# smallflyingpig/speech-to-image-translation-without-text

Measured on AMD Instinct MI355X. Metric: StackGAN-v2 3-stage G+D train-step images/sec at 256px, higher is better.
Workload: dtype f32

## Files before the change

include/s2i_hip.h:

```cpp
#ifndef S2I_HIP_H
#define S2I_HIP_H

#include <stddef.h>
#include <stdint.h>

#ifdef __cplusplus
extern "C" {
#endif

#define S2I_ABI_VERSION 4

#define S2I_CONV_K1      0
#define S2I_CONV_K3S1    1
#define S2I_CONV_K4S2    2
#define S2I_TCONV_K4S2   3

#define S2I_CONV_1D      4

#define S2I_ACT_NONE     0
#define S2I_ACT_GLU      1
#define S2I_ACT_LRELU    2
#define S2I_ACT_TANH     3
#define S2I_ACT_RELU     4

// ... 145 lines not shown
                    long long* num_batches_tracked , float momentum,
                    float eps, float* out4, void* stream);
int s2i_bn_eval_coeffs(int C, const float* gamma, const float* beta, const float* running_mean,
                       const float* running_var, float eps, float* out4, void* stream);
int s2i_bn_act_forward(const float* y, long long M, int groups, int C, const float* coef4, int act,
                       const float* residual, float* out, void* stream);
int s2i_colstats(const float* y, long long M, int C, int ldy, float* part, int nparts,
                 void* stream);
int s2i_bn_act_bwd_reduce(const float* y, const float* dout, int lddout, long long M, int groups, int C,
                          const float* coef4, int act, float* part, int nparts, void* stream);
int s2i_bn_bwd_finalize(const float* part, int nparts, int groups, int C, long long count, float* dgamma,
                        float* dbeta, int accumulate, float* red2, void* stream);
int s2i_bn_act_bwd_apply(const float* y, const float* dout, int lddout, long long M, int groups, int C,
                         const float* coef4, const float* red2, int act, float* dy, void* stream);

int s2i_act_backward(const float* out, const float* dout, int lddout, long long M, int C, int act,
                     float* dy, void* stream);
int s2i_glu_forward(const float* x, long long M, int C, float* out, void* stream);
int s2i_glu_backward(const float* x, const float* dout, long long M, int C, float* dx,
                     void* stream);

int s2i_nchw_to_nhwc(const float* src, float* dst, int B, int C, int H, int W, int Cp,
                     void* stream);
int s2i_nhwc_to_nchw(const float* src, int lds, float* dst, int B, int C, int H, int W,
                     void* stream);
int s2i_image_to_u8(const float* src, int lds, unsigned char* dst, long long npix, void* stream);
int s2i_u8_to_image(const unsigned char* src, float* dst, int B, int H, int W, void* stream);
int s2i_image_batch(const unsigned char* pool, long long pool_bytes, const long long* offsets, const int* sizes,
                    int npool, const int* plan, int n, int S, int L, const int* tab1, const int* tab2, float* out0,
                    float* out1, float* out2, void* stream);
// ... 112 lines not shown
```

speech_to_image_translation_without_text_amd/_lib.py:

```python
import ctypes
import os

import torch

_HERE = os.path.dirname(os.path.abspath(__file__))
LIB_PATH = os.path.join(_HERE, "libs2i_hip.so")

CONV_K1, CONV_K3S1, CONV_K4S2, TCONV_K4S2, CONV_1D = 0, 1, 2, 3, 4
ACT_NONE, ACT_GLU, ACT_LRELU, ACT_TANH, ACT_RELU = 0, 1, 2, 3, 4
PACK_PLAIN, PACK_UPFOLD = 0, 1
DT_F32, DT_BF16 = 0, 1
POOL_MAX3S2, POOL_AVG3S1, POOL_GLOBAL = 0, 1, 2
POOL_THEN_LRN, LRN_THEN_POOL = 0, 1
LOGMEL_BFT, LOGMEL_NHWC = 0, 1
LOGMEL_TILE_FRAMES = 64
ABI_VERSION = 4

c_int, c_float, c_void_p, c_size_t, c_ll = (ctypes.c_int, ctypes.c_float, ctypes.c_void_p,
                                            ctypes.c_size_t, ctypes.c_longlong)


class ConvDesc(ctypes.Structure):
    _fields_ = [(n, c_int) for n in ("kind", "B", "H", "W", "Cx", "Cc", "N", "wmode", "flip", "wR",
                                     "ldw", "act", "stats", "ldy", "groups", "nosplit", "kw", "stride", "pad",
# ... 63 lines not shown
    "s2i_cvec_bias_table": (c_int, [P, P, c_int, c_int, c_int, c_int, c_int, P, P, c_size_t, P]),
    "s2i_border_sums_workspace_bytes": (c_size_t, [c_int, c_int, c_int, c_int]),
    "s2i_tap_sums": (c_int, [P, c_int, c_int, c_int, c_int, P, P, c_size_t, P]),
    "s2i_cvec_grads": (c_int, [P, P, P, c_int, c_int, c_int, c_int, c_int, c_int, c_int, P, P, c_int, P]),
    "s2i_wgrad_workspace_bytes": (c_size_t, [ctypes.POINTER(WgradDesc)]),
    "s2i_conv_wgrad": (c_int, [ctypes.POINTER(WgradDesc), P, P, P, P, P, c_size_t, P]),
    "s2i_pack_conv_weight": (c_int, [P, P, c_int, c_int, c_int, c_int, c_int, c_int, P]),
    "s2i_pack_conv_weights_batched": (c_int, [P, c_int, c_int, c_int, P]),
    "s2i_bn_finalize": (c_int, [P, c_int, c_int, c_int, c_ll, P, P, P, P, P, c_float, c_float, P, P]),
    "s2i_bn_eval_coeffs": (c_int, [c_int, P, P, P, P, c_float, P, P]),
    "s2i_bn_act_forward": (c_int, [P, c_ll, c_int, c_int, P, c_int, P, P, P]),
    "s2i_colstats": (c_int, [P, c_ll, c_int, c_int, P, c_int, P]),
    "s2i_bn_act_bwd_reduce": (c_int, [P, P, c_int, c_ll, c_int, c_int, P, c_int, P, c_int, P]),
    "s2i_bn_bwd_finalize": (c_int, [P, c_int, c_int, c_int, c_ll, P, P, c_int, P, P]),
    "s2i_bn_act_bwd_apply": (c_int, [P, P, c_int, c_ll, c_int, c_int, P, P, c_int, P, P]),
    "s2i_act_backward": (c_int, [P, P, c_int, c_ll, c_int, c_int, P, P]),
    "s2i_glu_forward": (c_int, [P, c_ll, c_int, P, P]),
    "s2i_glu_backward": (c_int, [P, P, c_ll, c_int, P, P]),
    "s2i_nchw_to_nhwc": (c_int, [P, P, c_int, c_int, c_int, c_int, c_int, P]),
    "s2i_nhwc_to_nchw": (c_int, [P, c_int, P, c_int, c_int, c_int, c_int, P]),
    "s2i_image_to_u8": (c_int, [P, c_int, P, c_ll, P]),
    "s2i_u8_to_image": (c_int, [P, P, c_int, c_int, c_int, P]),
    "s2i_image_batch": (c_int, [P, c_ll, P, P, c_int, P, c_int, c_int, c_int, P, P, P, P, P, P]),
    "s2i_spatial_sum": (c_int, [P, c_int, c_int, c_int, c_int, P, P, c_size_t, P]),
    "s2i_spatial_sum_workspace_bytes": (c_size_t, [c_int, c_int, c_int]),
    "s2i_reparam_forward": (c_int, [P, P, c_int, c_int, P, P]),
    "s2i_reparam_backward": (c_int, [P, P, P, P, P, c_int, c_int, P, P]),
    "s2i_kl_forward": (c_int, [P, c_int, P, c_int, c_int, c_int, P, P]),
    "s2i_kl_backward": (c_int, [P, c_int, P, c_int, c_int, c_int, P, P, P, P]),
    "s2i_logit_forward": (c_int, [P, P, P, c_int, c_int, P, P]),
# ... 56 lines not shown
        fn = getattr(lib, name)
        fn.restype = res
        fn.argtypes = args
    if lib.s2i_version() != ABI_VERSION:
        raise S2IError("libs2i_hip.so ABI version %d, expected %d: rebuild it (make -C csrc)" % (lib.s2i_version(), ABI_VERSION))
    _lib = lib
    return lib


def check(rc, what):
    if rc != 0:
        msg = load().s2i_last_error()
        raise S2IError("%s failed: %s" % (what, msg.decode() if msg else "unknown error"))


class tuning:

    def __init__(self, **knobs):
        self.knobs = knobs

    def __enter__(self):
        lib = load()
        self.old = {}
        for k, v in self.knobs.items():
            cur = c_int(0)
            check(lib.s2i_get_tuning(k.encode(), ctypes.byref(cur)), "s2i_get_tuning")
            self.old[k] = cur.value
            check(lib.s2i_set_tuning(k.encode(), int(v)), "s2i_set_tuning")
        return self

    def __exit__(self, *exc):
        lib = load()
        for k, v in self.old.items():
            check(lib.s2i_set_tuning(k.encode(), v), "s2i_set_tuning")
        return False


def require_device():
    global _device_checked
    if _device_checked:
        return
    if not torch.cuda.is_available():
        raise S2IError("no HIP device visible: the MI355X kernels have no CPU fallback")
    check(load().s2i_check_device(), "s2i_check_device")
    _device_checked = True


def ptr(t):
    if t is None:
# ... 15 lines not shown
```

speech_to_image_translation_without_text_amd/csrc/s2i_bn.hip:

```cpp
#include "s2i_elementwise.h"

namespace {
template <typename T>
__device__ __forceinline__ f32x4 act_dz(const T* __restrict__ y, const T* __restrict__ dout, int lddout,
                                        long long row, int C, int quad, const float* __restrict__ coef,
                                        int act, f32x4 yv) {
  const float* scale = coef + 2 * C;
  const float* shift = coef + 3 * C;
  f32x4 dz;
  if (act == S2I_ACT_GLU) {
    const int hq = C / 8;
    const bool first = quad < hq;
    const int pq = first ? quad + hq : quad - hq;
    const f32x4 yp = ld4(y + row * C + pq * 4);
    const f32x4 d = ld4(dout + row * lddout + (first ? quad : pq) * 4);
    const f32x4 sa = ld4(scale + (first ? quad : pq) * 4), ta = ld4(shift + (first ? quad : pq) * 4);
    const f32x4 sg = ld4(scale + (first ? pq : quad) * 4), tg = ld4(shift + (first ? pq : quad) * 4);
    const f32x4 ya = first ? yv : yp, yg = first ? yp : yv;
#pragma unroll
    for (int j = 0; j < 4; ++j) {
      const float za = sa[j] * ya[j] + ta[j];
      const float sgm = sigmoid_gate_<T>(sg[j] * yg[j] + tg[j]);
      dz[j] = first ? d[j] * sgm : d[j] * za * sgm * (1.f - sgm);
    }
// ... 752 lines not shown
  }
}
}
extern "C" int s2i_glu_forward(const float* x, long long M, int C, float* out, void* stream) {
  S2I_REQUIRE(x && out && M > 0 && C > 0 && C % 2 == 0, "glu_forward: bad args");
  hipLaunchKernelGGL(glu_fwd_kernel, dim3(grid_for(M * (C / 2))), dim3(256), 0, ST, x, M, C, out);
  S2I_LAUNCH_CHECK("glu_forward");
  return 0;
}
extern "C" int s2i_glu_backward(const float* x, const float* dout, long long M, int C, float* dx, void* stream) {
  S2I_REQUIRE(x && dout && dx && M > 0 && C > 0 && C % 2 == 0, "glu_backward: bad args");
  hipLaunchKernelGGL(glu_bwd_kernel, dim3(grid_for(M * (C / 2))), dim3(256), 0, ST, x, dout, M, C, dx);
  S2I_LAUNCH_CHECK("glu_backward");
  return 0;
}
```

speech_to_image_translation_without_text_amd/csrc/s2i_common.h:

```cpp
#pragma once
#include <hip/hip_runtime.h>
#include <stdio.h>
#include <stdarg.h>
#include "../../include/s2i_hip.h"

typedef float f32x16 __attribute__((ext_vector_type(16)));
typedef float f32x4 __attribute__((ext_vector_type(4)));

void s2i_set_error(const char* fmt, ...);

#define S2I_FAIL(...)            \
  do {                           \
    s2i_set_error(__VA_ARGS__);  \
    return 1;                    \
  } while (0)

#define S2I_REQUIRE(cond, ...)   \
  do {                           \
    if (!(cond)) S2I_FAIL(__VA_ARGS__); \
  } while (0)

#define S2I_LAUNCH_CHECK(name)                                          \
  do {                                                                  \
    hipError_t e__ = hipGetLastError();                                 \
// ... 5 lines not shown
  while ((1 << l) < v) ++l;
  return l;
}
static inline bool s2i_is_pow2(int v) { return v > 0 && (v & (v - 1)) == 0; }
static inline int s2i_cdiv(long long a, long long b) { return (int)((a + b - 1) / b); }

enum {
  S2I_TUNE_FWD_BM = 0,
  S2I_TUNE_FWD_MIN_CPS,
  S2I_TUNE_B16_V2,
  S2I_TUNE_B16_PERSIST,
  S2I_TUNE_FINALIZE_THREADS,
  S2I_TUNE_B16_DBG,
  S2I_TUNE_WGRAD16_BM,
  S2I_TUNE_WGRAD_BM,
  S2I_TUNE_COUNT
};
int s2i_tune(int key, int def);
```

speech_to_image_translation_without_text_amd/csrc/s2i_conv.hip:

```cpp
#include "s2i_igemm.h"

namespace {

static int fwd_splitk(long long blocks, int nchunks, int nosplit, int min_cps) {
  int splitk = 1;
  if (blocks < 512 && nchunks >= 16 && !nosplit) {
    splitk = (int)(768 / blocks);
    if (splitk > nchunks / min_cps) splitk = nchunks / min_cps;
    if (splitk > 64) splitk = 64;
    if (splitk < 1) splitk = 1;
  }
  return splitk;
}

int plan_fwd(const s2i_conv_desc* d, FwdPlan* pl) {
  S2I_REQUIRE(d->B > 0 && d->H > 0 && d->W > 0 && d->N > 0, "conv: non-positive extent");
  S2I_REQUIRE(d->Cx >= 0 && d->Cc >= 0 && (d->Cx % 4) == 0 && (d->Cc % 4) == 0 && d->Cx + d->Cc > 0,
              "conv: channel counts must be multiples of 4 (Cx=%d Cc=%d)", d->Cx, d->Cc);
  S2I_REQUIRE(s2i_is_pow2(d->H) && s2i_is_pow2(d->W), "conv: spatial extents must be powers of two");
  pl->Ca = d->Cx + d->Cc;
  pl->nphases = 1;
  switch (d->kind) {
    case S2I_CONV_K1: pl->T = 1; pl->Ho = d->H; pl->Wo = d->W; break;
    case S2I_CONV_K3S1: pl->T = 9; pl->Ho = d->H; pl->Wo = d->W; break;
// ... 83 lines not shown
    if (ppg < 1) ppg = 1;
    return ppg * groups;
  }
  return pl.gridM * pl.nphases;
}

extern "C" int s2i_conv_stat_parts(const s2i_conv_desc* d) {
  FwdPlan pl;
  if (plan_fwd(d, &pl)) return -1;
  return stat_parts_for(pl, d->groups);
}

static int conv_forward_impl(const s2i_conv_desc* d, const float* x, const float* cvec, const float* w,
                             const unsigned short* wsp, int planes, int np, int kp, const float* bias,
                             const float* cls_bias, float* y, float* part, void* ws, size_t ws_bytes, void* stream,
                             int x16 = 0, int y16 = 0, const float* in_coef = nullptr) {
  FwdPlan pl;
  if (plan_fwd(d, &pl)) return 1;
  S2I_REQUIRE(!cls_bias || (d->kind == S2I_CONV_K3S1 && pl.splitk == 1), "conv: class bias needs an unsplit 3x3 conv");
  S2I_REQUIRE(x != nullptr || d->Cx == 0, "conv: x is null");
  S2I_REQUIRE(d->Cc == 0 || cvec != nullptr, "conv: cvec is null but Cc > 0");
  S2I_REQUIRE((w || wsp) && y, "conv: null weight/output");
  S2I_REQUIRE(!d->stats || part, "conv: stats requested without a partial buffer");
  const size_t need = pl.splitk > 1 ? (size_t)pl.splitk * pl.Mrows * d->N * sizeof(float) : 0;
  S2I_REQUIRE(ws_bytes >= need && (need == 0 || ws), "conv: workspace too small (%zu < %zu)", ws_bytes, need);
  hipStream_t st = (hipStream_t)stream;
  IgemmP p;
  p.x = x; p.cvec = cvec; p.w = w; p.bias = bias; p.cls_bias = cls_bias; p.y = y; p.part = part; p.slab = (float*)ws;
  p.B = d->B; p.H = d->H; p.W = d->W; p.Cx = d->Cx; p.Cc = d->Cc; p.Ca = pl.Ca;
  p.Ho = pl.Ho; p.Wo = pl.Wo; p.lgWo = s2i_ilog2(pl.Wo); p.lgHoWo = s2i_ilog2(pl.Ho * pl.Wo);
  p.M = pl.M; p.N = d->N; p.K = pl.K; p.T = pl.T;
// ... 33 lines not shown
  S2I_REQUIRE(xb < 0x7ff00000ull && wb < 0x7ff00000ull, "conv: tensor exceeds the 2 GiB buffer-addressing window");
  p.x_bytes = (unsigned)xb;
  p.c_bytes = (unsigned)((unsigned long long)d->B * d->Cc * 4ull);
  p.w_bytes = (unsigned)wb;
  const bool ca32 = (pl.Ca % 32) == 0 && (d->Cc % 32) == 0;
  if (wsp) {
    const unsigned long long pe = (unsigned long long)wtaps * np * kp;
    S2I_REQUIRE(pe * planes * 2ull < 0x7ff00000ull, "conv(split): weight planes exceed the buffer window");
    S2I_REQUIRE(kp >= pl.Ca && np >= d->N, "conv(split): weight planes %d x %d too small for N=%d K=%d", np, kp, d->N, pl.Ca);
    p.wsp_plane = (int)pe;
    p.wsp_bytes = (unsigned)(pe * planes * 2ull);
    if (launch_igemm_fwd_split(pl, p, grid, planes, st)) return 1;
  } else {
    if (launch_igemm_fwd(pl, p, grid, wt, ca32, st)) return 1;
  }
  if (pl.splitk > 1) return launch_splitk_reduce(d, pl, bias, y, part, ws, y16, stream);
  return 0;
}

extern "C" int s2i_conv_forward(const s2i_conv_desc* d, const float* x, const float* cvec, const float* w,
                                const float* bias, float* y, float* part, void* ws, size_t ws_bytes,
                                void* stream) {
  return s2i_conv_forward_cls(d, x, cvec, w, bias, nullptr, y, part, ws, ws_bytes, stream);
}

extern "C" int s2i_conv_forward_cls(const s2i_conv_desc* d, const float* x, const float* cvec, const float* w,
                                    const float* bias, const float* cls_bias, float* y, float* part, void* ws,
                                    size_t ws_bytes, void* stream) {
  S2I_REQUIRE(w != nullptr, "conv: null weight");
  return conv_forward_impl(d, x, cvec, w, nullptr, 0, 0, 0, bias, cls_bias, y, part, ws, ws_bytes, stream);
}

// ... 34 lines not shown
```

speech_to_image_translation_without_text_amd/csrc/s2i_runtime.hip:

```cpp
#include "s2i_common.h"
#include <string.h>

static thread_local char g_err[512] = "";

void s2i_set_error(const char* fmt, ...) {
  va_list ap;
  va_start(ap, fmt);
  vsnprintf(g_err, sizeof(g_err), fmt, ap);
  va_end(ap);
}

extern "C" const char* s2i_last_error(void) { return g_err; }

extern "C" int s2i_version(void) { return S2I_ABI_VERSION; }

extern "C" int s2i_check_device(void) {
  int dev = 0;
  hipError_t e = hipGetDevice(&dev);
  if (e != hipSuccess) S2I_FAIL("check_device: hipGetDevice: %s", hipGetErrorString(e));
  hipDeviceProp_t prop;
  e = hipGetDeviceProperties(&prop, dev);
  if (e != hipSuccess) S2I_FAIL("check_device: hipGetDeviceProperties: %s", hipGetErrorString(e));
  if (strncmp(prop.gcnArchName, "gfx950", 6) != 0)
    S2I_FAIL("check_device: kernels are built for gfx950 only, device %d is %s", dev, prop.gcnArchName);
  return 0;
}

#include <stdlib.h>
static const char* const g_tune_names[S2I_TUNE_COUNT] = {"fwd_bm", "fwd_min_cps", "b16_v2", "b16_persist", "finalize_threads", "b16_dbg",
                                                            "wgrad16_bm", "wgrad_bm"};
static int g_tune_val[S2I_TUNE_COUNT];
static bool g_tune_set[S2I_TUNE_COUNT];

static int tune_index(const char* key, size_t len) {
  for (int i = 0; i < S2I_TUNE_COUNT; ++i)
    if (strlen(g_tune_names[i]) == len && strncmp(g_tune_names[i], key, len) == 0) return i;
  return -1;
}

namespace {
struct TuneInit {
  TuneInit() {
    const char* e = getenv("S2I_TUNE");
    while (e && *e) {
      const char* eq = strchr(e, '=');
// ... 27 lines not shown
```

speech_to_image_translation_without_text_amd/ops.py:

```python
import ctypes
import os

import torch

from . import _lib
from ._lib import (ACT_GLU, ACT_LRELU, ACT_NONE, CONV_K1, CONV_K3S1, CONV_K4S2, DT_BF16, DT_F32,
                   PACK_PLAIN, PACK_UPFOLD, TCONV_K4S2, ConvDesc, WgradDesc, check, ptr, stream)

BN_EPS = 1e-5
BN_MOMENTUM = 0.1

DIRECT_PARAM_GRAD = False


def _direct(p):
    return (DIRECT_PARAM_GRAD and p is not None and p.requires_grad and p.grad is not None
            and p.grad.is_contiguous())


class param_grad_mode:

    def __init__(self, direct=True):
        self.new = bool(direct)

# ... 455 lines not shown
        expect = ld
        for dim in range(t.dim() - 2, -1, -1):
            if t.shape[dim] != 1 and st[dim] != expect:
                ok = False
                break
            expect *= t.shape[dim]
        if ok:
            return t, ld
    return t.contiguous(), C


def _num_parts(M):
    return int(max(1, min(1024, M // 64)))


_KIND = {"k1": CONV_K1, "k3s1": CONV_K3S1, "k4s2": CONV_K4S2, "up": TCONV_K4S2}


_DGRAD = {"k3s1": (CONV_K3S1, 1), "k4s2": (TCONV_K4S2, 0), "up": (CONV_K4S2, 0), "k1": (CONV_K1, 0)}


def _dgrad(kind_name, dy, w, packed, n_in, out_dtype=None):
    Op = packed.shape[2]
    if dy.shape[-1] != Op:
        raise _lib.S2IError("dgrad: dy has %d channels, packed weight %d" % (dy.shape[-1], Op))
    if out_dtype is not None:
        kind, flip = _DGRAD[kind_name]
        return conv_any(kind, dy, packed, n_in, wmode=1, flip=flip, out_dtype=out_dtype)[0]
    if kind_name == "k3s1":
        y, _, _ = conv_raw(CONV_K3S1, dy, None, packed, n_in, wmode=1, flip=1, wR=packed.shape[1], ldw=Op)
# ... 74 lines not shown
            else:
                real(x)
                in_src = None
        x = x.contiguous()
        if cvec is not None:
            cvec = cvec.contiguous()
        kind = _KIND[kind_name]
        packed = packed_weight(weight, PACK_UPFOLD if kind_name == "up" else PACK_PLAIN)
        Cout = weight.shape[0]
        factored = _factor_cvec(kind_name, cvec, x)
        bf = (ACT_BF16 and kind_name != "k1") or x.dtype == torch.bfloat16
        if bf and in_src is not None:
            raise _lib.S2IError("ConvBnAct: apply-on-load input in the bf16 activation mode")
        adt = torch.bfloat16 if bf else torch.float32
        cat_cc = 0
        if bf and cvec is not None and not factored:
            B_, H_, W_, _ = x.shape
            cat_cc = cvec.shape[1]
            x = torch.cat((cast(cvec, adt).view(B_, 1, 1, cat_cc).expand(B_, H_, W_, cat_cc), cast(x, adt)), 3).contiguous()
            cvec_used = None
        else:
            cvec_used = cvec
        if factored:
            B, Cc = cvec.shape
            Ip, Op = packed.shape[1], packed.shape[2]
            table = torch.empty((B, 9, Cout), dtype=torch.float32, device=x.device)
            ws = _ws.get(B * 9 * Cout * 4, x.device)
            check(lib.s2i_cvec_bias_table(ptr(cvec), ptr(packed), B, Cc, Ip, Op, Cout, ptr(table), ptr(ws),
                                          ws.numel() * 4, stream()), "s2i_cvec_bias_table")
            if bf:
                y, part, nparts = conv_any(kind, x, packed, Cout, stats=training, groups=groups, w_offset=Cc * Op,
                                           cls_bias=table, out_dtype=adt)
            else:
                y, part, nparts = conv_raw(kind, x, None, packed, Cout, wR=Ip, ldw=Op, stats=training, groups=groups,
                                           w_offset=Cc * Op, cls_bias=table)
        elif bf:
            y, part, nparts = conv_any(kind, x, packed, Cout, stats=training, groups=groups, out_dtype=adt)
        else:
            y, part, nparts = conv_raw(kind, x, cvec, packed, Cout, wR=packed.shape[1], ldw=packed.shape[2],
                                       stats=training, groups=groups, in_src=in_src)
        M = y.numel() // Cout
        if not training:
            groups = 1
        coef = torch.empty((groups, 4, Cout), dtype=torch.float32, device=x.device)
        rm, rv, nbt = bn_buffers
        if training:
            check(lib.s2i_bn_finalize(ptr(part), nparts, groups, Cout, M // groups, ptr(gamma), ptr(beta), ptr(rm),
                                      ptr(rv), ptr(nbt), BN_MOMENTUM, BN_EPS, ptr(coef), stream()), "s2i_bn_finalize")
        else:
            check(lib.s2i_bn_eval_coeffs(Cout, ptr(gamma), ptr(beta), ptr(rm), ptr(rv), BN_EPS, ptr(coef), stream()),
                  "s2i_bn_eval_coeffs")
        Cact = Cout // 2 if act == ACT_GLU else Cout
        out = torch.empty(y.shape[:-1] + (Cact,), dtype=adt, device=x.device)
        if residual is not None:
            residual = cast(real(residual), adt).contiguous()
        if defer and DEFER_ACT and training and act == ACT_LRELU and residual is None and not bf and not MATH_PLANES:
            out._s2i_lazy = _Lazy(y, coef, act, groups)
        else:
            check(lib.s2i_bn_act_forward_dt(_dt(y), ptr(y), M, groups, Cout, ptr(coef), act, ptr(residual), ptr(out),
                                            stream()), "s2i_bn_act_forward")
        ctx.save_for_backward(x, cvec_used, weight, gamma, y, coef, None if in_src is None else in_src.coef)
        ctx.in_src = None if in_src is None else (in_src.act, in_src.groups)
        ctx.beta_ref = beta
        ctx.kind_name, ctx.act, ctx.training, ctx.has_res = kind_name, act, training, residual is not None
        ctx.groups = groups
        ctx.factored = factored
        ctx.bf, ctx.cat_cc = bf, cat_cc
        return out

    @staticmethod
    def backward(ctx, dout):
        lib = _lib_ready()
        x, cvec, weight, gamma, y, coef, in_coef = ctx.saved_tensors
        if not ctx.training:
            raise _lib.S2IError("ConvBnAct.backward: eval-mode BatchNorm has no backward on this path")
        a_src = None
        if ctx.in_src is not None:
            a_src = _Lazy(x, in_coef, ctx.in_src[0], ctx.in_src[1])
        Cout = weight.shape[0]
        M = y.numel() // Cout
        if dout.dtype != y.dtype:
            dout = cast(dout, y.dtype)
        dout_k, ldd = _rows_view(dout)
        G = ctx.groups
        nparts = _num_parts(M // G) * G
        part = torch.empty((2, nparts, Cout), dtype=torch.float32, device=y.device)
        check(lib.s2i_bn_act_bwd_reduce_dt(_dt(y), ptr(y), ptr(dout_k), ldd, M, G, Cout, ptr(coef), ctx.act, ptr(part),
                                           nparts, stream()), "s2i_bn_act_bwd_reduce")
        beta = ctx.beta_ref
        need_gb = ctx.needs_input_grad[3] or ctx.needs_input_grad[4]
        direct_bn = need_gb and _direct(gamma) and _direct(beta)
        if not need_gb:
            dgamma = dbeta = None
        else:
            dgamma = gamma.grad if direct_bn else torch.empty_like(gamma)
            dbeta = beta.grad if direct_bn else torch.empty_like(gamma)
        red2 = torch.empty((G, 2, Cout), dtype=torch.float32, device=y.device)
        check(lib.s2i_bn_bwd_finalize(ptr(part), nparts, G, Cout, M // G, ptr(dgamma), ptr(dbeta),
                                      1 if direct_bn else 0, ptr(red2), stream()), "s2i_bn_bwd_finalize")
        if direct_bn:
            dgamma = dbeta = None
        dy = torch.empty_like(y)
        check(lib.s2i_bn_act_bwd_apply_dt(_dt(y), ptr(y), ptr(dout_k), ldd, M, G, Cout, ptr(coef), ptr(red2), ctx.act,
                                          ptr(dy), stream()), "s2i_bn_act_bwd_apply")
        need_x, need_c, need_w = ctx.needs_input_grad[0], ctx.needs_input_grad[1], ctx.needs_input_grad[2]
        dx = dc = dw = None
        Cc = 0 if cvec is None else cvec.shape[1]
        bf = ctx.bf
        if bf and not ctx.factored:
            cc = ctx.cat_cc
            if need_x or (need_c and cc):
                packed = packed_weight(weight, PACK_UPFOLD if ctx.kind_name == "up" else PACK_PLAIN)
                dx_full = _dgrad(ctx.kind_name, dy, weight, packed, x.shape[-1], out_dtype=x.dtype)
                dx, dc = _split_input_grad(dx_full, cc)
                if not need_x:
                    dx = None
                if not need_c:
                    dc = None
            if need_w:
# ... 407 lines not shown
```

Measured before the change: 786.5.

## Fuse BN stats, finalize and activation into single column kernels for small layers

Adds column-parallel BatchNorm kernels where each block owns a channel slice and loops over all rows of a group. In the forward pass the conv split-K slab reduction, statistics, coefficient finalize, running-stat update and activation run in one launch. In the backward pass the reduce, finalize and apply steps run in one launch. This targets launch overhead and partial-sum round trips on small-M layers, which the 3-stage StackGAN has many of. The cost is lower parallelism, since few blocks each cover many rows, plus extra eligibility branching, and it only applies when rows per group fall under a tunable limit.

```diff
diff --git a/include/s2i_hip.h b/include/s2i_hip.h
--- a/include/s2i_hip.h
+++ b/include/s2i_hip.h
@@ -183,6 +183,22 @@
 int s2i_bn_act_bwd_apply(const float* y, const float* dout, int lddout, long long M, int groups, int C,
                          const float* coef4, const float* red2, int act, float* dy, void* stream);
 
+int s2i_conv_bn_column_rows(void);
+int s2i_bn_column_forward(const float* slab, int S, long long M, int groups, int C, int nparts, float* y,
+                          const float* gamma, const float* beta, float* running_mean, float* running_var,
+                          long long* num_batches_tracked, float momentum, float eps, float* coef4, int act,
+                          const float* residual, float* out, void* stream);
+int s2i_bn_column_backward(const float* y, const float* dout, int lddout, long long M, int groups, int C,
+                           const float* coef4, int act, int nparts, float* dgamma, float* dbeta, int accumulate,
+                           float* red2, float* dy, void* stream);
+int s2i_conv_bn_column_eligible(const s2i_conv_desc* d);
+int s2i_conv_forward_bn_column(const s2i_conv_desc* d, const float* x, const float* cvec, const float* w,
+                               const unsigned short* wsplit, int planes, int np, int kp, const float* cls_bias,
+                               float* y, void* ws, size_t ws_bytes, const float* gamma, const float* beta,
+                               float* running_mean, float* running_var, long long* num_batches_tracked,
+                               float momentum, float eps, float* coef4, int act, const float* residual,
+                               float* out, void* stream);
+
 int s2i_act_backward(const float* out, const float* dout, int lddout, long long M, int C, int act,
                      float* dy, void* stream);
 int s2i_glu_forward(const float* x, long long M, int C, float* out, void* stream);
diff --git a/speech_to_image_translation_without_text_amd/_lib.py b/speech_to_image_translation_without_text_amd/_lib.py
--- a/speech_to_image_translation_without_text_amd/_lib.py
+++ b/speech_to_image_translation_without_text_amd/_lib.py
@@ -101,6 +101,12 @@
     "s2i_bn_act_bwd_reduce": (c_int, [P, P, c_int, c_ll, c_int, c_int, P, c_int, P, c_int, P]),
     "s2i_bn_bwd_finalize": (c_int, [P, c_int, c_int, c_int, c_ll, P, P, c_int, P, P]),
     "s2i_bn_act_bwd_apply": (c_int, [P, P, c_int, c_ll, c_int, c_int, P, P, c_int, P, P]),
+    "s2i_conv_bn_column_rows": (c_int, []),
+    "s2i_bn_column_forward": (c_int, [P, c_int, c_ll, c_int, c_int, c_int, P, P, P, P, P, P, c_float, c_float, P, c_int, P, P, P]),
+    "s2i_bn_column_backward": (c_int, [P, P, c_int, c_ll, c_int, c_int, P, c_int, c_int, P, P, c_int, P, P, P]),
+    "s2i_conv_bn_column_eligible": (c_int, [ctypes.POINTER(ConvDesc)]),
+    "s2i_conv_forward_bn_column": (c_int, [ctypes.POINTER(ConvDesc), P, P, P, P, c_int, c_int, c_int, P, P, P, c_size_t, P, P, P, P,
+                                           P, c_float, c_float, P, c_int, P, P, P]),
     "s2i_act_backward": (c_int, [P, P, c_int, c_ll, c_int, c_int, P, P]),
     "s2i_glu_forward": (c_int, [P, c_ll, c_int, P, P]),
     "s2i_glu_backward": (c_int, [P, P, c_ll, c_int, P, P]),
@@ -187,6 +193,9 @@
         raise S2IError("%s failed: %s" % (what, msg.decode() if msg else "unknown error"))
 
 
+tuning_generation = [0]
+
+
 class tuning:
 
     def __init__(self, **knobs):
@@ -200,12 +209,14 @@
             check(lib.s2i_get_tuning(k.encode(), ctypes.byref(cur)), "s2i_get_tuning")
             self.old[k] = cur.value
             check(lib.s2i_set_tuning(k.encode(), int(v)), "s2i_set_tuning")
+        tuning_generation[0] += 1
         return self
 
     def __exit__(self, *exc):
         lib = load()
         for k, v in self.old.items():
             check(lib.s2i_set_tuning(k.encode(), v), "s2i_set_tuning")
+        tuning_generation[0] += 1
         return False
 
 
diff --git a/speech_to_image_translation_without_text_amd/csrc/s2i_bn.hip b/speech_to_image_translation_without_text_amd/csrc/s2i_bn.hip
--- a/speech_to_image_translation_without_text_amd/csrc/s2i_bn.hip
+++ b/speech_to_image_translation_without_text_amd/csrc/s2i_bn.hip
@@ -790,3 +790,354 @@
   S2I_LAUNCH_CHECK("glu_backward");
   return 0;
 }
+
+struct ColGeom { int rpb, qpb, lgq, nslots, grid; };
+static ColGeom col_geom(int C, bool glu) {
+  const RedGeom r = red_geom(C);
+  ColGeom g;
+  g.rpb = r.rpb;
+  int qpb = r.cpb < 16 ? r.cpb : 16;
+  while (qpb > 4 && (r.Q + qpb - 1) / qpb < 64) qpb >>= 1;
+  g.qpb = qpb;
+  g.lgq = s2i_ilog2(qpb);
+  g.nslots = r.cpb / qpb;
+  g.grid = glu ? (r.Q / 2 + qpb / 2 - 1) / (qpb / 2) : (r.Q + qpb - 1) / qpb;
+  return g;
+}
+
+namespace {
+struct ColThread { int ql, il, lane, slot, quad; bool live; };
+template <bool GLU> __device__ __forceinline__ ColThread col_thread(int C, int lgq, int rpb) {
+  ColThread t;
+  const int qpb = 1 << lgq;
+  t.ql = threadIdx.x & (qpb - 1);
+  t.il = threadIdx.x >> lgq;
+  t.lane = t.il % rpb;
+  t.slot = t.il / rpb;
+  if (GLU) {
+    const int h = qpb >> 1, hq = C / 8;
+    const int vq = blockIdx.x * h + (t.ql & (h - 1));
+    t.live = vq < hq;
+    t.quad = t.ql < h ? vq : vq + hq;
+  } else {
+    t.quad = blockIdx.x * qpb + t.ql;
+    t.live = t.quad < C / 4;
+  }
+  return t;
+}
+
+__device__ __forceinline__ void col_round(f32x4 (*sh)[256], const ColThread& t, int qpb, int rpb, bool has, f32x4 s0,
+                                          f32x4 s1, double (&a)[8]) {
+  sh[0][threadIdx.x] = s0;
+  sh[1][threadIdx.x] = s1;
+  __syncthreads();
+  if (t.lane == 0 && has) {
+    for (int r = 1; r < rpb; ++r) {
+      s0 += sh[0][(t.slot * rpb + r) * qpb + t.ql];
+      s1 += sh[1][(t.slot * rpb + r) * qpb + t.ql];
+    }
+#pragma unroll
+    for (int j = 0; j < 4; ++j) { a[j] += s0[j]; a[4 + j] += s1[j]; }
+  }
+  __syncthreads();
+}
+__device__ __forceinline__ void col_total(f32x4 (*sh)[256], const ColThread& t, int qpb, int nslots, double (&a)[8]) {
+  double* shd = reinterpret_cast<double*>(sh);
+#pragma unroll
+  for (int half = 0; half < 2; ++half) {
+    if (t.lane == 0 && t.slot > 0) {
+#pragma unroll
+      for (int j = 0; j < 4; ++j) shd[(t.slot * qpb + t.ql) * 4 + j] = a[half * 4 + j];
+    }
+    __syncthreads();
+    if (t.il == 0) {
+      for (int s = 1; s < nslots; ++s)
+#pragma unroll
+        for (int j = 0; j < 4; ++j) a[half * 4 + j] += shd[(s * qpb + t.ql) * 4 + j];
+    }
+    __syncthreads();
+  }
+}
+
+template <int ACT>
+__global__ __launch_bounds__(256) void bn_column_fwd_kernel(const float* __restrict__ slab, int S, int G, int Rg, int C,
+                                                            int ppg, float* y, double count,
+                                                            const float* __restrict__ gamma, const float* __restrict__ beta,
+                                                            float* __restrict__ rmean, float* __restrict__ rvar,
+                                                            long long* __restrict__ nbt, float momentum, float eps,
+                                                            float* __restrict__ coef0, const float* __restrict__ residual,
+                                                            float* __restrict__ out, int lgq, int rpb, int nslots) {
+  constexpr bool GLU = ACT == S2I_ACT_GLU;
+  __shared__ f32x4 sh[2][256];
+  __shared__ f32x4 shc[2][16];
+  const int qpb = 1 << lgq, L = 256 >> lgq;
+  const ColThread t = col_thread<GLU>(C, lgq, rpb);
+  if (nbt && blockIdx.x == 0 && threadIdx.x == 0) nbt[0] += G;
+  const size_t sstride = (size_t)G * Rg * C;
+  const int chunk = (Rg + ppg - 1) / ppg;
+  float rm[4] = {0.f, 0.f, 0.f, 0.f}, rv[4] = {0.f, 0.f, 0.f, 0.f};
+  if (t.il == 0 && t.live && rmean) {
+#pragma unroll
+    for (int j = 0; j < 4; ++j) { rm[j] = rmean[t.quad * 4 + j]; rv[j] = rvar[t.quad * 4 + j]; }
+  }
+  for (int g = 0; g < G; ++g) {
+    const long long g0 = (long long)g * Rg, gend = g0 + Rg;
+    double a[8] = {0, 0, 0, 0, 0, 0, 0, 0};
+    for (int c0 = 0; c0 < ppg; c0 += nslots) {
+      const int pp = c0 + t.slot;
+      const bool has = t.live && pp < ppg;
+      f32x4 s0 = {0.f, 0.f, 0.f, 0.f}, s1 = {0.f, 0.f, 0.f, 0.f};
+      if (has) {
+        const long long r0 = g0 + (long long)pp * chunk;
+        const long long r1 = r0 + chunk < gend ? r0 + chunk : gend;
+        for (long long row = r0 + t.lane; row < r1; row += rpb) {
+          const float* sp = slab + row * C + t.quad * 4;
+          f32x4 v = *reinterpret_cast<const f32x4*>(sp);
+          for (int s = 1; s < S; ++s) v += *reinterpret_cast<const f32x4*>(sp + s * sstride);
+          *reinterpret_cast<f32x4*>(y + row * C + t.quad * 4) = v;
+          s0 += v;
+          s1 += v * v;
+        }
+      }
+      col_round(sh, t, qpb, rpb, has, s0, s1, a);
+    }
+    col_total(sh, t, qpb, nslots, a);
+    if (t.il == 0 && t.live) {
+      float* o = coef0 + (size_t)g * 4 * C;
+      f32x4 scv, shv;
+#pragma unroll
+      for (int j = 0; j < 4; ++j) {
+        const int c = t.quad * 4 + j;
+        const double a0 = a[j], a1 = a[4 + j];
+        const double mean = a0 / count;
+        double var = a1 / count - mean * mean;
+        if (var < 0) var = 0;
+        const float invstd = (float)(1.0 / sqrt(var + (double)eps));
+        const float sc = gamma[c] * invstd;
+        o[c] = (float)mean;
+        o[C + c] = invstd;
+        o[2 * C + c] = sc;
+        o[3 * C + c] = beta[c] - (float)mean * sc;
+        scv[j] = sc;
+        shv[j] = o[3 * C + c];
+        const double unb = count > 1 ? var * count / (count - 1) : var;
+        if (ppg <= 8) {
+          rm[j] = __builtin_fmaf(1.f - momentum, rm[j], momentum * (float)mean);
+          rv[j] = __builtin_fmaf(1.f - momentum, rv[j], momentum * (float)unb);
+        } else {
+          rm[j] = __builtin_fmaf(momentum, (float)mean, (1.f - momentum) * rm[j]);
+          rv[j] = __builtin_fmaf(momentum, (float)unb, (1.f - momentum) * rv[j]);
+        }
+      }
+      shc[0][t.ql] = scv;
+      shc[1][t.ql] = shv;
+    }
+    __syncthreads();
+    if (t.live) {
+      if (GLU) {
+        const int h = qpb >> 1, lq = t.ql & (h - 1), Cout = C / 2;
+        const int vq = blockIdx.x * h + lq;
+        const f32x4 sa = shc[0][lq], ta = shc[1][lq], sg = shc[0][lq + h], tg = shc[1][lq + h];
+        for (long long row = g0 + t.il + (t.ql < h ? 0 : L); row < gend; row += 2 * L) {
+          const f32x4 ya = ld4(y + row * C + vq * 4), yg = ld4(y + row * C + Cout + vq * 4);
+          f32x4 o;
+#pragma unroll
+          for (int j = 0; j < 4; ++j) o[j] = (sa[j] * ya[j] + ta[j]) * sigmoid_gate_<float>(sg[j] * yg[j] + tg[j]);
+          st4(out + row * Cout + vq * 4, o);
+        }
+      } else {
+        const f32x4 sc = shc[0][t.ql], shf = shc[1][t.ql];
+        auto one = [&](long long row, const f32x4& yv, const f32x4& rs) {
+          f32x4 o;
+#pragma unroll
+          for (int j = 0; j < 4; ++j) {
+            float z = sc[j] * yv[j] + shf[j];
+            if (ACT == S2I_ACT_LRELU) z = z > 0.f ? z : 0.2f * z;
+            o[j] = z;
+          }
+          if (residual) o += rs;
+          st4(out + row * C + t.quad * 4, o);
+        };
+        long long row = g0 + t.il;
+        for (; row + 3 * L < gend; row += 4 * L) {
+          f32x4 yv[4], rs[4];
+#pragma unroll
+          for (int u = 0; u < 4; ++u) {
+            yv[u] = ld4(y + (row + u * L) * C + t.quad * 4);
+            rs[u] = residual ? ld4(residual + (row + u * L) * C + t.quad * 4) : yv[u];
+          }
+#pragma unroll
+          for (int u = 0; u < 4; ++u) one(row + u * L, yv[u], rs[u]);
+        }
+        for (; row < gend; row += L) {
+          const f32x4 yv = ld4(y + row * C + t.quad * 4);
+          one(row, yv, residual ? ld4(residual + row * C + t.quad * 4) : yv);
+        }
+      }
+    }
+    __syncthreads();
+  }
+  if (t.il == 0 && t.live && rmean) {
+#pragma unroll
+    for (int j = 0; j < 4; ++j) { rmean[t.quad * 4 + j] = rm[j]; rvar[t.quad * 4 + j] = rv[j]; }
+  }
+}
+
+template <int ACT>
+__global__ __launch_bounds__(256) void bn_column_bwd_kernel(const float* __restrict__ y, const float* __restrict__ dout,
+                                                            int lddout, int G, int Rg, int C, int ppg,
+                                                            const float* __restrict__ coef0, double count,
+                                                            float* __restrict__ dgamma, float* __restrict__ dbeta,
+                                                            int accumulate, float* __restrict__ red20,
+                                                            float* __restrict__ dy, int lgq, int rpb, int nslots) {
+  constexpr int RPT = 4;
+  __shared__ f32x4 sh[2][256];
+  __shared__ f32x4 shc[2][16];
+  const int qpb = 1 << lgq, L = 256 >> lgq;
+  const ColThread t = col_thread<false>(C, lgq, rpb);
+  const long long M = (long long)G * Rg;
+  const int chunk = (Rg + ppg - 1) / ppg;
+  double gs0[4] = {0, 0, 0, 0}, gs1[4] = {0, 0, 0, 0};
+  for (int g = 0; g < G; ++g) {
+    const long long g0 = (long long)g * Rg, gend = g0 + Rg;
+    const float* coef = coef0 + (size_t)g * 4 * C;
+    f32x4 mean = {0.f, 0.f, 0.f, 0.f}, invstd = mean, sc = mean, shf = mean;
+    if (t.live) {
+      mean = ld4(coef + t.quad * 4); invstd = ld4(coef + C + t.quad * 4);
+      sc = ld4(coef + 2 * C + t.quad * 4); shf = ld4(coef + 3 * C + t.quad * 4);
+    }
+    double a[8] = {0, 0, 0, 0, 0, 0, 0, 0};
+    for (int c0 = 0; c0 < ppg; c0 += nslots) {
+      const int pp = c0 + t.slot;
+      const bool has = t.live && pp < ppg;
+      f32x4 s0 = {0.f, 0.f, 0.f, 0.f}, s1 = {0.f, 0.f, 0.f, 0.f};
+      if (has) {
+        const long long r0 = g0 + (long long)pp * chunk;
+        const long long r1 = r0 + chunk < gend ? r0 + chunk : gend;
+        long long row = r0 + t.lane;
+        for (; row + (RPT - 1) * rpb < r1; row += RPT * rpb) {
+          f32x4 yv[RPT], dz[RPT];
+#pragma unroll
+          for (int u = 0; u < RPT; ++u) yv[u] = ld4(y + (row + u * rpb) * C + t.quad * 4);
+#pragma unroll
+          for (int u = 0; u < RPT; ++u) dz[u] = act_dz(y, dout, lddout, row + u * rpb, C, t.quad, coef, ACT, yv[u]);
+#pragma unroll
+          for (int u = 0; u < RPT; ++u) {
+            s0 += dz[u];
+            s1 += dz[u] * ((yv[u] - mean) * invstd);
+          }
+        }
+        for (; row < r1; row += rpb) {
+          const f32x4 yv = ld4(y + row * C + t.quad * 4);
+          const f32x4 dz = act_dz(y, dout, lddout, row, C, t.quad, coef, ACT, yv);
+          s0 += dz;
+          s1 += dz * ((yv - mean) * invstd);
+        }
+      }
+      col_round(sh, t, qpb, rpb, has, s0, s1, a);
+    }
+    col_total(sh, t, qpb, nslots, a);
+    if (t.il == 0 && t.live) {
+      float* o = red20 + (size_t)g * 2 * C;
+      f32x4 m0v, m1v;
+#pragma unroll
+      for (int j = 0; j < 4; ++j) {
+        const int c = t.quad * 4 + j;
+        o[c] = (float)(a[j] / count);
+        o[C + c] = (float)(a[4 + j] / count);
+        m0v[j] = o[c];
+        m1v[j] = o[C + c];
+        gs0[j] += a[j];
+        gs1[j] += a[4 + j];
+      }
+      shc[0][t.ql] = m0v;
+      shc[1][t.ql] = m1v;
+    }
+    __syncthreads();
+    if (t.live) {
+      const f32x4 m0 = shc[0][t.ql], m1 = shc[1][t.ql];
+      auto finish = [&](long long row, const f32x4& yv, const f32x4& d) {
+        f32x4 o;
+#pragma unroll
+        for (int j = 0; j < 4; ++j) {
+          float dz;
+          if (ACT == S2I_ACT_LRELU) dz = (sc[j] * yv[j] + shf[j]) > 0.f ? d[j] : 0.2f * d[j];
+          else dz = d[j];
+          const float xh = (yv[j] - mean[j]) * invstd[j];
+          o[j] = sc[j] * (dz - m0[j] - xh * m1[j]);
+        }
+        st4(dy + row * C + t.quad * 4, o);
+      };
+      long long row = g0 + t.il;
+      for (; row + (RPT - 1) * L < gend; row += RPT * L) {
+        f32x4 yv[RPT], d[RPT];
+#pragma unroll
+        for (int u = 0; u < RPT; ++u) {
+          yv[u] = ld4(y + (row + u * L) * C + t.quad * 4);
+          d[u] = ld4(dout + (row + u * L) * lddout + t.quad * 4);
+        }
+#pragma unroll
+        for (int u = 0; u < RPT; ++u) finish(row + u * L, yv[u], d[u]);
+      }
+      for (; row < gend; row += L) finish(row, ld4(y + row * C + t.quad * 4), ld4(dout + row * lddout + t.quad * 4));
+    }
+    __syncthreads();
+  }
+  (void)M;
+  if (t.il == 0 && t.live) {
+#pragma unroll
+    for (int j = 0; j < 4; ++j) {
+      const int c = t.quad * 4 + j;
+      if (dbeta) dbeta[c] = accumulate ? dbeta[c] + (float)gs0[j] : (float)gs0[j];
+      if (dgamma) dgamma[c] = accumulate ? dgamma[c] + (float)gs1[j] : (float)gs1[j];
+    }
+  }
+}
+}
+
+extern "C" int s2i_conv_bn_column_rows(void) { return s2i_tune(S2I_TUNE_BN_COLUMN_ROWS, S2I_BN_COLUMN_ROWS_DEFAULT); }
+
+extern "C" int s2i_bn_column_forward(const float* slab, int S, long long M, int groups, int C, int nparts, float* y,
+                                     const float* gamma, const float* beta, float* running_mean, float* running_var,
+                                     long long* num_batches_tracked, float momentum, float eps, float* coef4, int act,
+                                     const float* residual, float* out, void* stream) {
+  S2I_REQUIRE(slab && y && gamma && beta && coef4 && out && S >= 1 && M > 0 && C > 0, "bn_column_forward: bad args");
+  S2I_REQUIRE(act == S2I_ACT_NONE || act == S2I_ACT_GLU || act == S2I_ACT_LRELU,
+              "bn_column_forward: activation %d is not NONE, GLU or LRELU", act);
+  S2I_REQUIRE(groups >= 1 && M % groups == 0 && M < (1ll << 31) && nparts > 0 && nparts % groups == 0,
+              "bn_column_forward: bad grouping");
+  S2I_REQUIRE(act == S2I_ACT_GLU ? C % 8 == 0 : C % 4 == 0, "bn_column_forward: C=%d not aligned for act %d", C, act);
+  S2I_REQUIRE(!(residual && act == S2I_ACT_GLU), "bn_column_forward: residual with GLU unsupported");
+  S2I_REQUIRE((running_mean == nullptr) == (running_var == nullptr), "bn_column_forward: running stats must come in pairs");
+  const ColGeom g = col_geom(C, act == S2I_ACT_GLU);
+  const int Rg = (int)(M / groups);
+#define S2I_COLF(ACTV) hipLaunchKernelGGL((bn_column_fwd_kernel<ACTV>), dim3(g.grid), dim3(256), 0, ST, slab, S, groups, Rg, C, \
+                                          nparts / groups, y, (double)Rg, gamma, beta, running_mean, running_var,                \
+                                          num_batches_tracked, momentum, eps, coef4, residual, out, g.lgq, g.rpb, g.nslots)
+  if (act == S2I_ACT_GLU) S2I_COLF(S2I_ACT_GLU);
+  else if (act == S2I_ACT_LRELU) S2I_COLF(S2I_ACT_LRELU);
+  else S2I_COLF(S2I_ACT_NONE);
+#undef S2I_COLF
+  S2I_LAUNCH_CHECK("bn_column_forward");
+  return 0;
+}
+
+extern "C" int s2i_bn_column_backward(const float* y, const float* dout, int lddout, long long M, int groups, int C,
+                                      const float* coef4, int act, int nparts, float* dgamma, float* dbeta, int accumulate,
+                                      float* red2, float* dy, void* stream) {
+  S2I_REQUIRE(y && dout && coef4 && red2 && dy && M > 0 && C > 0 && C % 4 == 0, "bn_column_backward: bad args");
+  S2I_REQUIRE(act == S2I_ACT_NONE || act == S2I_ACT_LRELU, "bn_column_backward: activation %d is not NONE or LRELU", act);
+  S2I_REQUIRE(groups >= 1 && M % groups == 0 && M < (1ll << 31) && nparts > 0 && nparts % groups == 0,
+              "bn_column_backward: bad grouping");
+  S2I_REQUIRE(lddout % 4 == 0 && lddout >= C, "bn_column_backward: lddout alignment");
+  const ColGeom g = col_geom(C, false);
+  const int Rg = (int)(M / groups);
+#define S2I_COLB(ACTV) hipLaunchKernelGGL((bn_column_bwd_kernel<ACTV>), dim3(g.grid), dim3(256), 0, ST, y, dout, lddout, groups, \
+                                          Rg, C, nparts / groups, coef4, (double)Rg, dgamma, dbeta, accumulate, red2, dy, g.lgq,   \
+                                          g.rpb, g.nslots)
+  if (act == S2I_ACT_LRELU) S2I_COLB(S2I_ACT_LRELU);
+  else S2I_COLB(S2I_ACT_NONE);
+#undef S2I_COLB
+  S2I_LAUNCH_CHECK("bn_column_backward");
+  return 0;
+}
diff --git a/speech_to_image_translation_without_text_amd/csrc/s2i_common.h b/speech_to_image_translation_without_text_amd/csrc/s2i_common.h
--- a/speech_to_image_translation_without_text_amd/csrc/s2i_common.h
+++ b/speech_to_image_translation_without_text_amd/csrc/s2i_common.h
@@ -43,6 +43,8 @@
   S2I_TUNE_B16_DBG,
   S2I_TUNE_WGRAD16_BM,
   S2I_TUNE_WGRAD_BM,
+  S2I_TUNE_BN_COLUMN_ROWS,
   S2I_TUNE_COUNT
 };
+#define S2I_BN_COLUMN_ROWS_DEFAULT 0
 int s2i_tune(int key, int def);
diff --git a/speech_to_image_translation_without_text_amd/csrc/s2i_conv.hip b/speech_to_image_translation_without_text_amd/csrc/s2i_conv.hip
--- a/speech_to_image_translation_without_text_amd/csrc/s2i_conv.hip
+++ b/speech_to_image_translation_without_text_amd/csrc/s2i_conv.hip
@@ -121,7 +121,7 @@
 static int conv_forward_impl(const s2i_conv_desc* d, const float* x, const float* cvec, const float* w,
                              const unsigned short* wsp, int planes, int np, int kp, const float* bias,
                              const float* cls_bias, float* y, float* part, void* ws, size_t ws_bytes, void* stream,
-                             int x16 = 0, int y16 = 0, const float* in_coef = nullptr) {
+                             int x16 = 0, int y16 = 0, const float* in_coef = nullptr, int* slabs = nullptr) {
   FwdPlan pl;
   if (plan_fwd(d, &pl)) return 1;
   S2I_REQUIRE(!cls_bias || (d->kind == S2I_CONV_K3S1 && pl.splitk == 1), "conv: class bias needs an unsplit 3x3 conv");
@@ -185,8 +185,50 @@
   } else {
     if (launch_igemm_fwd(pl, p, grid, wt, ca32, st)) return 1;
   }
+  if (slabs) {
+    *slabs = pl.splitk > 1 ? pl.splitk : 0;
+    return 0;
+  }
   if (pl.splitk > 1) return launch_splitk_reduce(d, pl, bias, y, part, ws, y16, stream);
   return 0;
+}
+
+static bool column_fwd_ok(const s2i_conv_desc* d, const FwdPlan& pl) {
+  const int groups = d->groups < 1 ? 1 : d->groups;
+  const int cap = s2i_conv_bn_column_rows();
+  return d->stats && pl.splitk > 1 && (d->N % 4) == 0 && d->ldy == d->N && d->act == S2I_ACT_NONE &&
+         (pl.Mrows % groups) == 0 && pl.Mrows / groups <= cap;
+}
+
+extern "C" int s2i_conv_bn_column_eligible(const s2i_conv_desc* d) {
+  FwdPlan pl;
+  if (plan_fwd(d, &pl)) return 0;
+  return column_fwd_ok(d, pl) ? 1 : 0;
+}
+
+extern "C" int s2i_conv_forward_bn_column(const s2i_conv_desc* d, const float* x, const float* cvec, const float* w,
+                                          const unsigned short* wsplit, int planes, int np, int kp, const float* cls_bias,
+                                          float* y, void* ws, size_t ws_bytes, const float* gamma, const float* beta,
+                                          float* running_mean, float* running_var, long long* num_batches_tracked,
+                                          float momentum, float eps, float* coef4, int act, const float* residual,
+                                          float* out, void* stream) {
+  FwdPlan pl;
+  if (plan_fwd(d, &pl)) return 1;
+  S2I_REQUIRE(column_fwd_ok(d, pl), "conv(bn_column): layer not eligible (s2i_conv_bn_column_eligible)");
+  S2I_REQUIRE((w != nullptr) != (wsplit != nullptr), "conv(bn_column): one of the fp32 weight and the bf16 planes");
+  if (wsplit) {
+    S2I_REQUIRE(planes >= 1 && planes <= 3 && np > 0 && kp > 0 && (kp % 8) == 0 && s2i_conv_split_eligible(d),
+                "conv(bn_column): bad bf16 planes");
+  }
+  int S = 0;
+  if (conv_forward_impl(d, x, cvec, w, wsplit, planes, np, kp, nullptr, cls_bias, y, coef4, ws, ws_bytes, stream, 0, 0,
+                        nullptr, &S))
+    return 1;
+  S2I_REQUIRE(S > 1, "conv(bn_column): the layer did not split");
+  const int groups = d->groups < 1 ? 1 : d->groups;
+  return s2i_bn_column_forward((const float*)ws, S, pl.Mrows, groups, d->N, stat_parts_for(pl, groups), y, gamma, beta,
+                               running_mean, running_var, num_batches_tracked, momentum, eps, coef4, act, residual, out,
+                               stream);
 }
 
 extern "C" int s2i_conv_forward(const s2i_conv_desc* d, const float* x, const float* cvec, const float* w,
diff --git a/speech_to_image_translation_without_text_amd/csrc/s2i_runtime.hip b/speech_to_image_translation_without_text_amd/csrc/s2i_runtime.hip
--- a/speech_to_image_translation_without_text_amd/csrc/s2i_runtime.hip
+++ b/speech_to_image_translation_without_text_amd/csrc/s2i_runtime.hip
@@ -28,7 +28,7 @@
 
 #include <stdlib.h>
 static const char* const g_tune_names[S2I_TUNE_COUNT] = {"fwd_bm", "fwd_min_cps", "b16_v2", "b16_persist", "finalize_threads", "b16_dbg",
-                                                            "wgrad16_bm", "wgrad_bm"};
+                                                            "wgrad16_bm", "wgrad_bm", "bn_column_rows"};
 static int g_tune_val[S2I_TUNE_COUNT];
 static bool g_tune_set[S2I_TUNE_COUNT];
 
diff --git a/speech_to_image_translation_without_text_amd/ops.py b/speech_to_image_translation_without_text_amd/ops.py
--- a/speech_to_image_translation_without_text_amd/ops.py
+++ b/speech_to_image_translation_without_text_amd/ops.py
@@ -493,6 +493,50 @@
     return int(max(1, min(1024, M // 64)))
 
 
+COLUMN_LOG = None
+_column_cap = [-1, 0]
+
+
+def column_rows(lib):
+    if _column_cap[0] != _lib.tuning_generation[0]:
+        _column_cap[0], _column_cap[1] = _lib.tuning_generation[0], lib.s2i_conv_bn_column_rows()
+    return _column_cap[1]
+
+
+def conv_bn_column(kind, x, cvec, packed, N, *, wR, ldw, groups, w_offset, cls_bias, gamma, beta, bn_buffers, act, residual):
+    lib = _lib_ready()
+    cap = column_rows(lib)
+    B, H, W, Cx = x.shape
+    Ho, Wo = _geom(kind, H, W)
+    g = groups if groups else 1
+    if cap <= 0 or (B * Ho * Wo) // g > cap or (residual is not None and act == ACT_GLU):
+        return None
+    Cc = 0 if cvec is None else cvec.shape[1]
+    d = ConvDesc(kind, B, H, W, Cx, Cc, N, 0, 0, wR, ldw, ACT_NONE, 1, N, groups, 1 if cls_bias is not None else 0, 0, 0, 0,
+                 128 if MATH_PLANES else TILE_ROWS, 0, 0)
+    if not lib.s2i_conv_bn_column_eligible(ctypes.byref(d)):
+        return None
+    y = torch.empty((B, Ho, Wo, N), dtype=torch.float32, device=x.device)
+    coef = torch.empty((g, 4, N), dtype=torch.float32, device=x.device)
+    out = torch.empty((B, Ho, Wo, N // 2 if act == ACT_GLU else N), dtype=torch.float32, device=x.device)
+    if EXEC_LOG is not None:
+        _log_exec("conv k%d [%d,%d,%d,%d+%d]->%d" % (kind, B, H, W, Cx, Cc, N), B * Ho * Wo, N, _TAPS[kind] * (Cx + Cc),
+                  x.numel(), _TAPS[kind] * (Cx + Cc) * N * (4 if kind == TCONV_K4S2 else 1), y.numel())
+    if COLUMN_LOG is not None:
+        COLUMN_LOG.append(("fwd", B * Ho * Wo, g, N))
+    ws = _ws.get(lib.s2i_conv_workspace_bytes(ctypes.byref(d)), x.device)
+    w, wsp, np_, kp = ptr(packed) + 4 * int(w_offset), None, 0, 0
+    if (MATH_PLANES and w_offset == 0 and packed.dim() == 3 and getattr(packed, '_s2i_gen', None) is not None
+            and lib.s2i_conv_split_eligible(ctypes.byref(d)) and packed.shape[1] % 8 == 0):
+        w, wsp, np_, kp = None, split_weight(packed, MATH_PLANES, True), packed.shape[2], packed.shape[1]
+    rm, rv, nbt = bn_buffers
+    check(lib.s2i_conv_forward_bn_column(ctypes.byref(d), ptr(x), ptr(cvec), w, ptr(wsp), MATH_PLANES if wsp is not None else 0,
+                                         np_, kp, ptr(cls_bias), ptr(y), ptr(ws), ws.numel() * 4, ptr(gamma), ptr(beta), ptr(rm),
+                                         ptr(rv), ptr(nbt), BN_MOMENTUM, BN_EPS, ptr(coef), act, ptr(residual), ptr(out),
+                                         stream()), "s2i_conv_forward_bn_column")
+    return y, coef, out
+
+
 _KIND = {"k1": CONV_K1, "k3s1": CONV_K3S1, "k4s2": CONV_K4S2, "up": TCONV_K4S2}
 
 
@@ -597,6 +641,8 @@
             raise _lib.S2IError("ConvBnAct: apply-on-load input in the bf16 activation mode")
         adt = torch.bfloat16 if bf else torch.float32
         cat_cc = 0
+        fused = None
+        lazy_out = bool(defer and DEFER_ACT and training and act == ACT_LRELU and residual is None and not bf and not MATH_PLANES)
         if bf and cvec is not None and not factored:
             B_, H_, W_, _ = x.shape
             cat_cc = cvec.shape[1]
@@ -604,6 +650,9 @@
             cvec_used = None
         else:
             cvec_used = cvec
+        if residual is not None:
+            residual = cast(real(residual), adt).contiguous()
+        table = None
         if factored:
             B, Cc = cvec.shape
             Ip, Op = packed.shape[1], packed.shape[2]
@@ -614,14 +663,35 @@
             if bf:
                 y, part, nparts = conv_any(kind, x, packed, Cout, stats=training, groups=groups, w_offset=Cc * Op,
                                            cls_bias=table, out_dtype=adt)
+            elif training and not lazy_out and (fused := conv_bn_column(kind, x, None, packed, Cout, wR=Ip, ldw=Op,
+                                                                        groups=groups,
+                                                                        w_offset=Cc * Op, cls_bias=table, gamma=gamma, beta=beta,
+                                                                        bn_buffers=bn_buffers, act=act,
+                                                                        residual=residual)) is not None:
+                pass
             else:
                 y, part, nparts = conv_raw(kind, x, None, packed, Cout, wR=Ip, ldw=Op, stats=training, groups=groups,
                                            w_offset=Cc * Op, cls_bias=table)
         elif bf:
             y, part, nparts = conv_any(kind, x, packed, Cout, stats=training, groups=groups, out_dtype=adt)
+        elif (training and in_src is None and not lazy_out
+              and (fused := conv_bn_column(kind, x, cvec, packed, Cout, wR=packed.shape[1], ldw=packed.shape[2], groups=groups,
+                                           w_offset=0, cls_bias=None, gamma=gamma, beta=beta, bn_buffers=bn_buffers, act=act,
+                                           residual=residual)) is not None):
+            pass
         else:
             y, part, nparts = conv_raw(kind, x, cvec, packed, Cout, wR=packed.shape[1], ldw=packed.shape[2],
                                        stats=training, groups=groups, in_src=in_src)
+        if fused is not None:
+            y, coef, out = fused
+            ctx.save_for_backward(x, cvec_used, weight, gamma, y, coef, None)
+            ctx.in_src = None
+            ctx.beta_ref = beta
+            ctx.kind_name, ctx.act, ctx.training, ctx.has_res = kind_name, act, training, residual is not None
+            ctx.groups = groups
+            ctx.factored = factored
+            ctx.bf, ctx.cat_cc = bf, cat_cc
+            return out
         M = y.numel() // Cout
         if not training:
             groups = 1
@@ -635,9 +705,7 @@
                   "s2i_bn_eval_coeffs")
         Cact = Cout // 2 if act == ACT_GLU else Cout
         out = torch.empty(y.shape[:-1] + (Cact,), dtype=adt, device=x.device)
-        if residual is not None:
-            residual = cast(real(residual), adt).contiguous()
-        if defer and DEFER_ACT and training and act == ACT_LRELU and residual is None and not bf and not MATH_PLANES:
+        if lazy_out:
             out._s2i_lazy = _Lazy(y, coef, act, groups)
         else:
             check(lib.s2i_bn_act_forward_dt(_dt(y), ptr(y), M, groups, Cout, ptr(coef), act, ptr(residual), ptr(out),
@@ -667,25 +735,35 @@
         dout_k, ldd = _rows_view(dout)
         G = ctx.groups
         nparts = _num_parts(M // G) * G
-        part = torch.empty((2, nparts, Cout), dtype=torch.float32, device=y.device)
-        check(lib.s2i_bn_act_bwd_reduce_dt(_dt(y), ptr(y), ptr(dout_k), ldd, M, G, Cout, ptr(coef), ctx.act, ptr(part),
-                                           nparts, stream()), "s2i_bn_act_bwd_reduce")
         beta = ctx.beta_ref
         need_gb = ctx.needs_input_grad[3] or ctx.needs_input_grad[4]
         direct_bn = need_gb and _direct(gamma) and _direct(beta)
+        column = (y.dtype == torch.float32 and a_src is None and ctx.act in (ACT_LRELU, ACT_NONE)
+                  and M // G <= column_rows(lib))
+        if not column:
+            part = torch.empty((2, nparts, Cout), dtype=torch.float32, device=y.device)
+            check(lib.s2i_bn_act_bwd_reduce_dt(_dt(y), ptr(y), ptr(dout_k), ldd, M, G, Cout, ptr(coef), ctx.act, ptr(part),
+                                               nparts, stream()), "s2i_bn_act_bwd_reduce")
         if not need_gb:
             dgamma = dbeta = None
         else:
             dgamma = gamma.grad if direct_bn else torch.empty_like(gamma)
             dbeta = beta.grad if direct_bn else torch.empty_like(gamma)
         red2 = torch.empty((G, 2, Cout), dtype=torch.float32, device=y.device)
-        check(lib.s2i_bn_bwd_finalize(ptr(part), nparts, G, Cout, M // G, ptr(dgamma), ptr(dbeta),
-                                      1 if direct_bn else 0, ptr(red2), stream()), "s2i_bn_bwd_finalize")
+        dy = torch.empty_like(y)
+        if column:
+            if COLUMN_LOG is not None:
+                COLUMN_LOG.append(("bwd", M, G, Cout))
+            check(lib.s2i_bn_column_backward(ptr(y), ptr(dout_k), ldd, M, G, Cout, ptr(coef), ctx.act, nparts, ptr(dgamma),
+                                             ptr(dbeta), 1 if direct_bn else 0, ptr(red2), ptr(dy), stream()),
+                  "s2i_bn_column_backward")
+        else:
+            check(lib.s2i_bn_bwd_finalize(ptr(part), nparts, G, Cout, M // G, ptr(dgamma), ptr(dbeta),
+                                          1 if direct_bn else 0, ptr(red2), stream()), "s2i_bn_bwd_finalize")
+            check(lib.s2i_bn_act_bwd_apply_dt(_dt(y), ptr(y), ptr(dout_k), ldd, M, G, Cout, ptr(coef), ptr(red2), ctx.act,
+                                              ptr(dy), stream()), "s2i_bn_act_bwd_apply")
         if direct_bn:
             dgamma = dbeta = None
-        dy = torch.empty_like(y)
-        check(lib.s2i_bn_act_bwd_apply_dt(_dt(y), ptr(y), ptr(dout_k), ldd, M, G, Cout, ptr(coef), ptr(red2), ctx.act,
-                                          ptr(dy), stream()), "s2i_bn_act_bwd_apply")
         need_x, need_c, need_w = ctx.needs_input_grad[0], ctx.needs_input_grad[1], ctx.needs_input_grad[2]
         dx = dc = dw = None
         Cc = 0 if cvec is None else cvec.shape[1]
```

New measurement: 784.0. Within noise of the previous version (-0.3%).
